# metagentools/VStrains

Measured on AMD Instinct MI355X. Metric: PE read pairs/sec through PE-link inference (GFA index + packed reads in HBM -> node_mat/short_mat), higher is better.
Workload: dtype u32

## Files before the change

vstrains_amd/csrc/vs_acc_tasks.h:

```cpp
#ifndef VS_ACC_TASKS_H
#define VS_ACC_TASKS_H
#include <stdint.h>

#include "vs_pe_plan.h"

#define VS_ACC_NODE 0u
#define VS_ACC_LEFT 1u
#define VS_ACC_RIGHT 2u

VS_PLAN_FN uint32_t vs_acc_pair_tasks(uint32_t nl, uint32_t nr) { return (nr ? nl : 0u) + ((nl + 1u) >> 1) + ((nr + 1u) >> 1); }

struct VsAccSegs {
    uint32_t p1, p2, e;
};
VS_PLAN_FN VsAccSegs vs_acc_fold(uint32_t n, uint32_t a) {
    const uint32_t a2 = n - 1u - a;
    if (a2 == a) return VsAccSegs{a, n, n};
    const bool a_first = ((0u - (n - a)) & 3u) <= ((0u - (a + 1u)) & 3u);
    return VsAccSegs{a_first ? a : a2, a_first ? a2 : a, n};
}
VS_PLAN_FN VsAccSegs vs_acc_task_segs(uint32_t kind, uint32_t a, uint32_t nl, uint32_t nr) {
    return kind == VS_ACC_NODE ? VsAccSegs{0u, nr, nr} : vs_acc_fold(kind == VS_ACC_LEFT ? nl : nr, a);
}
VS_PLAN_FN uint32_t vs_acc_turns(const VsAccSegs &s) {
    return s.p2 < s.e ? ((s.e - s.p1 + 3u) & ~3u) + (s.e - s.p2) : s.e - s.p1;
}
VS_PLAN_FN uint32_t vs_acc_partners(const VsAccSegs &s) { return (s.e - s.p1) + (s.e - s.p2); }

struct VsAccClass {
    uint32_t a0, cnt, turns;
};
VS_PLAN_FN VsAccClass vs_acc_fold_class(uint32_t n, uint32_t r) {
    const uint32_t a0 = (n - r) & 3u;
    const uint32_t pad_a = (0u - r) & 3u, pad_m = (r - n - 1u) & 3u;
    return VsAccClass{a0, ((n >> 1) + 3u - a0) >> 2, n + 1u + (pad_a <= pad_m ? pad_a : pad_m)};
}

VS_PLAN_FN uint16_t vs_acc_task_entry(uint32_t pair, uint32_t kind, uint32_t a) { return (uint16_t)(0x8000u | pair | kind << 6 | a << 8); }
VS_PLAN_FN uint32_t vs_acc_entry_pair(uint32_t w) { return w & 63u; }
VS_PLAN_FN uint32_t vs_acc_entry_kind(uint32_t w) { return (w >> 6) & 3u; }
VS_PLAN_FN uint32_t vs_acc_entry_a(uint32_t w) { return (w >> 8) & 31u; }

VS_PLAN_FN bool vs_acc_batch_fits(uint32_t tasks_incl, uint32_t cap) { return tasks_incl <= cap; }
inline uint32_t vs_acc_batch_cut(const uint32_t *tasks, uint32_t n, uint32_t first, uint32_t cap) {
    uint32_t incl = 0, last = first;
    while (last < n && vs_acc_batch_fits(incl + tasks[last], cap)) incl += tasks[last++];
    return last;
}

#endif
```

vstrains_amd/csrc/vs_api.hip:

```cpp
#include <stdarg.h>
#include <stdio.h>
#include <stdlib.h>
#include <string.h>

#include "vs_internal.h"

static thread_local std::string g_create_err;

int vs_fail(vs_ctx *ctx, int code, const char *fmt, ...) {
    char buf[512];
    va_list ap;
    va_start(ap, fmt);
    vsnprintf(buf, sizeof buf, fmt, ap);
    va_end(ap);
    if (ctx) ctx->err = buf; else g_create_err = buf;
    return code;
}

static bool env_on(const char *name) {
    const char *v = getenv(name);
    return v && atoi(v) != 0;
}

void vs_tuning_load(VsTuning &t, bool experiment) {
    t = VsTuning();
    if (!experiment) return;
    if (const char *v = getenv("VS_EPT")) t.ept = (uint32_t)atoi(v) & ~1u;
    if (const char *v = getenv("VS_GRID_PER_CU")) t.grid_per_cu = atoi(v) > 0 ? (uint32_t)atoi(v) : 128u;
    if (const char *v = getenv("VS_ACC_FILL")) t.acc_fill_pct = atoi(v);
    if (const char *v = getenv("VS_ACC_TASKS")) t.acc_tasks = atoi(v) > 0 ? (uint32_t)atoi(v) : 0u;
    if (const char *v = getenv("VS_SHORTCUT")) t.shortcut = atoi(v) != 0 ? 1 : 0;
    if (const char *v = getenv("VS_ADAPT_GRID")) t.adapt_grid = atoi(v) != 0 ? 1 : 0;
    if (const char *v = getenv("VS_ACC_ROWS")) t.acc_rows = atoi(v) != 0 ? 1 : 0;
    if (const char *v = getenv("VS_LTAB_BITS")) t.ltab_bits = atoi(v) >= 0 && atoi(v) <= 31 ? atoi(v) : -1;
    if (const char *v = getenv("VS_ROWS_KEYS")) t.rows_keys = atoi(v) >= 2 && atoi(v) <= 65536 ? (uint32_t)atoi(v) : 0u;
    if (const char *v = getenv("VS_ROWS_SUB")) t.rows_sub = atoi(v) >= 1024 ? (uint32_t)atoi(v) : 0u;
    if (const char *v = getenv("VS_ROWS_PER_STRIP")) t.rows_per_strip = atoi(v) > 0 && atoi(v) <= 64 ? (uint32_t)atoi(v) : 0u;
    t.no_sort = env_on("VS_NO_SORT");
    t.locus_global = env_on("VS_LOCUS_GLOBAL");
    t.no_fast = env_on("VS_NO_FAST");
    t.no_std = env_on("VS_NO_STD");
    t.no_agg = env_on("VS_NO_AGG");
    t.no_mid = env_on("VS_NO_MID");
}

extern "C" {

int vs_abi_version(void) { return VS_ABI_VERSION; }

int vs_device_count(void) {
    int n = 0;
    if (hipGetDeviceCount(&n) != hipSuccess) return 0;
    return n;
}

const char *vs_last_error(const vs_ctx *ctx) { return ctx ? ctx->err.c_str() : g_create_err.c_str(); }

int vs_ctx_create(int device, vs_ctx **out) {
    if (!out) return vs_fail(nullptr, VS_E_ARG, "vs_ctx_create: out is NULL");
    *out = nullptr;
    int n = 0;
    hipError_t e = hipGetDeviceCount(&n);
    if (e != hipSuccess || n <= 0)
        return vs_fail(nullptr, VS_E_HIP, "no HIP device available (%s); this library has no CPU path",
                       e == hipSuccess ? "device count 0" : hipGetErrorString(e));
    if (device < 0 || device >= n) return vs_fail(nullptr, VS_E_ARG, "device %d out of range (0..%d)", device, n - 1);
    e = hipSetDevice(device);
    if (e != hipSuccess) return vs_fail(nullptr, VS_E_HIP, "hipSetDevice(%d): %s", device, hipGetErrorString(e));
    vs_ctx *ctx = new vs_ctx();
    ctx->device = device;
    if (const char *ev = getenv("VS_EXPERIMENT")) ctx->experiment = strcmp(ev, "1") == 0;
    vs_tuning_load(ctx->tune, ctx->experiment);
    hipDeviceProp_t prop;
    if (hipGetDeviceProperties(&prop, device) == hipSuccess) ctx->n_cu = prop.multiProcessorCount;
    for (int i = 0; i < 5; i++) {
        e = hipEventCreate(&ctx->ev[i]);
        if (e != hipSuccess) {
            int rc = vs_fail(nullptr, VS_E_HIP, "hipEventCreate: %s", hipGetErrorString(e));
            delete ctx;
            return rc;
        }
    }
    *out = ctx;
// ... 162 lines not shown
```

vstrains_amd/csrc/vs_pe.hip:

```cpp
#include <stdio.h>
#include <stdlib.h>
#include <string.h>

#include <vector>

#include "vs_internal.h"
#include "vs_acc_tasks.h"
#include "vs_pe_pack.h"

#define TPB 256
#define LCAP 20u
__device__ __forceinline__ const uint32_t *vs_row_quad(const uint32_t *__restrict__ lists, const uint32_t *__restrict__ hi, uint64_t row, uint32_t q) {
    return q < LC / 4u ? lists + row * LC + 4u * q : hi + row * 4u;
}
#define EMPTY_NODE 0xFFFFFFFFu

struct PeParams {
    VsIndexDev idx;
    VsReadsDev rd;
    uint32_t *node_mat, *short_mat;
    unsigned long long *stats;
    uint32_t ept, pmax, words_cap, pool, pool_bits;
    uint64_t n_tiles;
    uint32_t *slow_list, *slow_count;
    uint32_t *dbg_lists, *dbg_counts;
    uint32_t dbg_cap;
    uint32_t accumulate;
    const uint32_t *perm;
    uint32_t wpe;
    uint32_t tiles_per_wg;
    uint32_t magic_pmax, magic_wpe;
    uint32_t *out_lists;
    uint32_t *out_counts;
    uint32_t out_rows;
    uint32_t *out_lists_hi;
    uint64_t n_pairs;
    uint32_t shortcut;
    uint8_t *tile_map;
    uint32_t tile_T;
    uint32_t mid_fast;
};

__device__ __forceinline__ void vs_mark_tile(uint8_t *map, uint32_t T, uint32_t mat, uint32_t x, uint32_t y) {
    if (!map) return;
    const uint64_t t = ((uint64_t)mat * T + (x >> 6)) * T + (y >> 6);
    if (!map[t]) map[t] = 1;
}

__device__ __forceinline__ void vs_mark_tile_store(uint8_t *map, uint32_t T, uint32_t mat, uint32_t x, uint32_t y) {
    if (map) map[((uint64_t)mat * T + (x >> 6)) * T + (y >> 6)] = 1;
}

struct Mem {
    uint32_t cnt, minp, minj;
};

struct __attribute__((packed, aligned(4))) VsQuad { uint32_t x, y, z, w; };

template <bool W4>
__device__ __forceinline__ void vs_agree_fast(const uint32_t *rw, uint32_t rbase, const uint32_t *tw, uint32_t tl, uint32_t cl,
// ... 756 lines not shown
                    P.out_counts[(uint64_t)tile * ept + i] = (s_state[i] & 3u) == 1u ? s_ns[i] : 0u;
            }
        }
        if (want_dbg) {
            for (uint32_t i = tid; i < ne; i += TTPB) {
                if (s_state[i] & 2u) continue;
                uint32_t n = s_ns[i];
                const uint64_t ge = s_gend[i];
                P.dbg_counts[ge] = n;
                for (uint32_t k2 = 0; k2 < n && k2 < P.dbg_cap; k2++) P.dbg_lists[ge * P.dbg_cap + k2] = s_list[s_off[i] + k2];
            }
        }
    }
    __syncthreads();
    if (tid < 3 && P.stats && s_misc[12 + tid]) atomicAdd(&P.stats[tid], (unsigned long long)s_misc[12 + tid]);
}

#define ACC_LDS_BYTES ((2u * ACC_SLOTS + (ACC_TPB / 64) * (ACC_TASK_WORDS + ACC_BINS) + 4u) * 4u)
static_assert(ACC_LDS_BYTES <= 160u * 1024u, "k_pe_accumulate: one workgroup per CU");
template <uint32_t BITS>
struct CellTable {
    static constexpr uint32_t EMPTY = 0xFFFFFFFFu;
    __device__ static uint32_t key(uint32_t mat, uint32_t x, uint32_t y, uint32_t N) { return (mat * N + x) * N + y; }
    __device__ static uint32_t slot(uint32_t k) { return ((((k >> 4) * 0x9E3779B1u) >> (36u - BITS)) << 4) | (k & 15u); }
    __device__ static uint32_t next(uint32_t at) { return (at + 16u) & ((1u << BITS) - 1u); }
};
typedef CellTable<ACC_BITS> Acc32;

template <typename TB>
__device__ __forceinline__ bool vs_cell_claim(uint32_t *s_key, uint32_t *s_cnt, uint32_t *s_used, uint32_t key, uint32_t at, uint32_t wgt) {
    for (uint32_t pr = 0; pr < 8u; pr++) {
        uint32_t kx = s_key[at];
        if (kx == TB::EMPTY) {
            kx = atomicCAS(&s_key[at], TB::EMPTY, key);
            if (kx == TB::EMPTY) { atomicAdd(s_used, 1u); kx = key; }
        }
        if (kx == key) {
            atomicAdd(&s_cnt[at], wgt);
            return true;
        }
        at = TB::next(at);
    }
    return false;
}

__device__ __forceinline__ void vs_wave_lds_sync() {
    __builtin_amdgcn_fence(__ATOMIC_RELEASE, "workgroup");
    __builtin_amdgcn_wave_barrier();
    __builtin_amdgcn_fence(__ATOMIC_ACQUIRE, "workgroup");
}

__global__ void __launch_bounds__(ACC_TPB)
k_pe_accumulate(const uint32_t *__restrict__ lists, const uint32_t *__restrict__ counts, uint64_t n_slots_pairs,
                uint32_t pairs_per_wg, uint32_t N, uint32_t use_table, uint32_t fill_limit, uint32_t task_cap,
                uint32_t *__restrict__ node_mat, uint32_t *__restrict__ short_mat, uint32_t *__restrict__ queue, uint32_t ept) {
    const uint32_t tid = threadIdx.x, lane = tid & 63u, wv = tid >> 6;
    uint32_t *s_key = vs_lds;
    uint32_t *s_cnt = vs_lds + ACC_SLOTS;
    uint32_t *s_bin = vs_lds + 2u * ACC_SLOTS + wv * (ACC_TASK_WORDS + ACC_BINS);
    uint16_t *s_task = (uint16_t *)(s_bin + ACC_BINS);
    uint32_t *s_misc = vs_lds + 2u * ACC_SLOTS + (ACC_TPB / 64) * (ACC_TASK_WORDS + ACC_BINS);
    uint32_t &s_used = s_misc[0], &s_lost = s_misc[1], &s_chunk = s_misc[2];
    const uint32_t NN = N * N;
    for (uint32_t i = tid; i < ACC_SLOTS; i += ACC_TPB) { s_key[i] = Acc32::EMPTY; s_cnt[i] = 0; }
    if (tid == 0) { s_used = 0; s_lost = 0; }
    __syncthreads();
    const uint32_t ppt = ept >> 1, region_q = (ept * LC) >> 2;
    auto write_out = [&]() {
        for (uint32_t i = tid; i < ACC_SLOTS; i += ACC_TPB) {
            const uint32_t key = s_key[i];
            if (key != Acc32::EMPTY) {
                atomicAdd(key >= NN ? short_mat + (key - NN) : node_mat + key, s_cnt[i]);
                s_key[i] = Acc32::EMPTY;
                s_cnt[i] = 0;
            }
        }
        if (tid == 0) { s_used = 0; s_lost = 0; }
        __syncthreads();
    };
    for (;;) {
    __syncthreads();
    if (tid == 0) s_chunk = atomicAdd(queue, 1u);
    __syncthreads();
    const uint64_t chunk = s_chunk;
    const uint64_t lo = chunk * pairs_per_wg;
    if (lo >= n_slots_pairs) break;
    const uint64_t hi = lo + pairs_per_wg < n_slots_pairs ? lo + pairs_per_wg : n_slots_pairs;
    for (uint64_t base = lo; base < hi; base += (ACC_TPB / 64u) * ACC_PPW) {
        const uint64_t wbase = base + wv * ACC_PPW;
        const uint32_t *wcounts = counts + 2u * wbase;
        const uint64_t tile0 = wbase / ppt;
        const uint32_t rem0 = (uint32_t)(wbase - tile0 * ppt);
        const uint32_t *wlists = lists + tile0 * ept * LC;
        uint32_t nl = 0, nr = 0, packed = 0;
        if (wbase + lane < hi) {
            const uint2 c = *(const uint2 *)(wcounts + 2u * lane);
            nl = c.x & 0xFFu; nr = c.y & 0xFFu;
            const uint32_t tq = (rem0 + lane) / ppt * region_q;
            packed = nl | nr << 5 | (tq + (c.x >> 8)) << 10 | (tq + (c.y >> 8)) << 21;
        }
        const uint32_t my_tasks = vs_acc_pair_tasks(nl, nr);
        for (uint32_t first = 0; first < ACC_PPW;) {
            const uint32_t incl = vs_wave_scan_add(lane >= first ? my_tasks : 0u);
            const uint32_t last = (uint32_t)__popcll(__ballot(vs_acc_batch_fits(incl, task_cap)));
            const uint32_t U = (uint32_t)__builtin_amdgcn_readlane((int)incl, (int)last - 1);
            const bool mine = lane >= first && lane < last;
            first = last;
            if (!U) continue;
            if (lane < ACC_BINS) s_bin[lane] = 0u;
            vs_wave_lds_sync();
            uint32_t o_n = 0, o_lm = 0, o_rm = 0, o_l[4], o_r[4];
            if (mine) {
                if (nl && nr) o_n = atomicAdd(&s_bin[nr], nl);
                if (nl & 1u) o_lm = atomicAdd(&s_bin[(nl + 1u) >> 1], 1u);
                if (nr & 1u) o_rm = atomicAdd(&s_bin[(nr + 1u) >> 1], 1u);
#pragma unroll
                for (uint32_t r = 0; r < 4u; r++) {
                    const VsAccClass cl = vs_acc_fold_class(nl, r), cr = vs_acc_fold_class(nr, r);
                    o_l[r] = cl.cnt ? atomicAdd(&s_bin[cl.turns], cl.cnt) : 0u;
                    o_r[r] = cr.cnt ? atomicAdd(&s_bin[cr.turns], cr.cnt) : 0u;
                }
            }
            vs_wave_lds_sync();
            {
                const uint32_t v = lane < ACC_BINS ? s_bin[ACC_BINS - 1u - lane] : 0u;
                const uint32_t before = vs_wave_scan_add(v) - v;
                if (lane < ACC_BINS) s_bin[ACC_BINS - 1u - lane] = before;
            }
            vs_wave_lds_sync();
            if (mine) {
                if (nl && nr) {
                    const uint32_t at = s_bin[nr] + o_n;
                    for (uint32_t a = 0; a < nl; a++) s_task[at + a] = vs_acc_task_entry(lane, VS_ACC_NODE, a);
                }
                if (nl & 1u) s_task[s_bin[(nl + 1u) >> 1] + o_lm] = vs_acc_task_entry(lane, VS_ACC_LEFT, nl >> 1);
                if (nr & 1u) s_task[s_bin[(nr + 1u) >> 1] + o_rm] = vs_acc_task_entry(lane, VS_ACC_RIGHT, nr >> 1);
                uint32_t nl2 = nl, nr2 = nr;
                asm volatile("" : "+v"(nl2), "+v"(nr2));
#pragma unroll
                for (uint32_t r = 0; r < 4u; r++) {
                    const VsAccClass cl = vs_acc_fold_class(nl2, r), cr = vs_acc_fold_class(nr2, r);
                    if (cl.cnt) {
                        const uint32_t at = s_bin[cl.turns] + o_l[r];
                        for (uint32_t i = 0; i < cl.cnt; i++) s_task[at + i] = vs_acc_task_entry(lane, VS_ACC_LEFT, cl.a0 + 4u * i);
                    }
                    if (cr.cnt) {
                        const uint32_t at = s_bin[cr.turns] + o_r[r];
                        for (uint32_t i = 0; i < cr.cnt; i++) s_task[at + i] = vs_acc_task_entry(lane, VS_ACC_RIGHT, cr.a0 + 4u * i);
                    }
                }
            }
            vs_wave_lds_sync();
            struct Task {
                uint32_t x, mat, off, p, p2, e, turns;
                VsQuad q;
            };
            auto decode = [&](uint32_t t0) {
                Task T;
                const uint32_t w = t0 + lane < U ? s_task[t0 + lane] : 0u;
                const uint32_t kind = vs_acc_entry_kind(w), a = vs_acc_entry_a(w);
                const uint32_t pk = __shfl(packed, (int)vs_acc_entry_pair(w), 64);
                const uint32_t ql = pk & 31u, qr = (pk >> 5) & 31u, rowl = ((pk >> 10) & 0x7FFu) << 2, rowr = (pk >> 21) << 2;
                const VsAccSegs s = w ? vs_acc_task_segs(kind, a, ql, qr) : VsAccSegs{0u, 0u, 0u};
                T.turns = vs_acc_turns(s);
                T.mat = kind != VS_ACC_NODE ? 1u : 0u;
                T.off = !w ? 0u : kind == VS_ACC_LEFT ? rowl : rowr;
                T.p = s.p1; T.p2 = s.p2; T.e = s.e;
                T.x = 0u;
                if (w && kind == VS_ACC_NODE) T.x = wlists[rowl + a];
                T.q = *(const VsQuad *)(wlists + T.off + T.p);
                return T;
            };
            Task nxt = decode(0u);
            for (uint32_t t0 = 0; t0 < U; t0 += 64u) {
                const Task c = nxt;
                if (t0 + 64u < U) nxt = decode(t0 + 64u);
                const uint32_t tmax = (uint32_t)__builtin_amdgcn_readlane((int)vs_wave_scan_max(c.turns), 63);
                const uint32_t mat = c.mat, e = c.e;
                const uint32_t *plist = wlists + c.off;
                uint32_t x = c.x, p = c.p, p2 = c.p2;
                bool fresh = true;
                VsQuad q = c.q;
                for (uint32_t t = 0; t < tmax; t += 4u) {
                    const uint32_t ys[4] = {q.x, q.y, q.z, q.w};
                    if (mat && fresh) x = ys[0];
                    const uint32_t pb = p;
                    p += 4u;
                    fresh = p >= e;
                    if (fresh) { p = p2; p2 = e; }
                    if (t + 4u < tmax) q = *(const VsQuad *)(plist + p);
                    const uint32_t left = tmax - t;
                    if (use_table) {
                        uint32_t key[4], seen[4], at[4];
#pragma unroll
                        for (uint32_t j = 0; j < 4u; j++) {
                            if (j >= left) break;
                            const uint32_t yv = ys[j];
                            const uint32_t cx = (mat && yv < x) ? yv : x, cy = (mat && yv < x) ? x : yv;
                            key[j] = Acc32::key(mat, cx, cy, N);
                            at[j] = Acc32::slot(key[j]);
                            seen[j] = s_key[at[j]];
                        }
#pragma unroll
                        for (uint32_t j = 0; j < 4u; j++) {
                            if (j >= left) break;
                            if (pb + j >= e) continue;
                            if (seen[j] == key[j]) {
                                atomicAdd(&s_cnt[at[j]], 1u);
                            } else if (!vs_cell_claim<Acc32>(s_key, s_cnt, &s_used, key[j], at[j], 1u)) {
                                atomicAdd(&s_lost, 1u);
                                atomicAdd(key[j] >= NN ? short_mat + (key[j] - NN) : node_mat + key[j], 1u);
                            }
                        }
                    } else {
#pragma unroll
                        for (uint32_t j = 0; j < 4u; j++) {
                            if (pb + j >= e) continue;
                            const uint32_t yv = ys[j];
                            const uint32_t cx = (mat && yv < x) ? yv : x, cy = (mat && yv < x) ? x : yv;
                            atomicAdd((mat ? short_mat : node_mat) + (uint64_t)cx * N + cy, 1u);
                        }
                    }
                }
            }
        }
        __syncthreads();
        const bool spill = s_used > fill_limit || s_lost > 4096u;
        __syncthreads();
        if (spill) write_out();
    }
    }
    __syncthreads();
    write_out();
}

__global__ void __launch_bounds__(256) k_mark_tiles(const uint32_t *__restrict__ lists, const uint32_t *__restrict__ counts,
                                                   uint64_t n_slots_pairs, uint8_t *__restrict__ map, uint32_t T, uint32_t ept) {
    const uint64_t p = (uint64_t)blockIdx.x * blockDim.x + threadIdx.x;
    if (p >= n_slots_pairs) return;
    const uint32_t cl = counts[2u * p], cr = counts[2u * p + 1u], nl = cl & 0xFFu, nr = cr & 0xFFu;
    if (!nl && !nr) return;
    const uint32_t *region = lists + 2u * p / ept * ept * LC, *rl = region + 4u * (cl >> 8), *rr = region + 4u * (cr >> 8);
    uint8_t *smap = map + (uint64_t)T * T;
    uint32_t tl[8], tr[8], kl = 0, kr = 0;
    bool over = false;
    auto put = [&](uint32_t (&tt)[8], uint32_t &k, uint32_t t) {
        bool seen = false;
#pragma unroll
        for (uint32_t j = 0; j < 8u; j++) seen |= j < k && tt[j] == t;
        if (seen) return;
        if (k >= 8u) { over = true; return; }
#pragma unroll
        for (uint32_t j = 0; j < 8u; j++)
            if (j == k) tt[j] = t;
        k++;
    };
#pragma unroll
    for (uint32_t j = 0; j < 8u; j++) { tl[j] = 0u; tr[j] = 0u; }
#pragma unroll
    for (uint32_t q = 0; q < LCAP / 4u; q++) {
        if (4u * q < nl) {
            const VsQuad v = *(const VsQuad *)(rl + 4u * q);
            const uint32_t e[4] = {v.x, v.y, v.z, v.w};
#pragma unroll
            for (uint32_t i = 0; i < 4u; i++)
                if (4u * q + i < nl) put(tl, kl, e[i] >> 6);
        }
        if (4u * q < nr) {
            const VsQuad v = *(const VsQuad *)(rr + 4u * q);
            const uint32_t e[4] = {v.x, v.y, v.z, v.w};
#pragma unroll
            for (uint32_t i = 0; i < 4u; i++)
                if (4u * q + i < nr) put(tr, kr, e[i] >> 6);
// ... 853 lines not shown
            for (uint32_t key_lo = 0; key_lo < N; key_lo += n_keys) {
                const uint32_t nk = N - key_lo < n_keys ? N - key_lo : n_keys;
                if (mode) hipLaunchKernelGGL(k_rows_count<1>, dim3(n_chunks1), dim3(ROWS_TPB), rl, st, sl, sh, sc, (const uint32_t *)owners, 0ull, (const uint32_t *)n_owners, key_lo, nk, row_count);
                else hipLaunchKernelGGL(k_rows_count<0>, dim3(n_chunks), dim3(ROWS_TPB), rl, st, sl, sh, sc, (const uint32_t *)nullptr, np, (const uint32_t *)nullptr, key_lo, nk, row_count);
            }
            int rc = vs_scan_u32(ctx, row_count, row_ptr, (uint64_t)N + 1u, scan_tmp, nullptr);
            if (rc) return rc;
            for (uint32_t key_lo = 0; key_lo < N; key_lo += n_keys) {
                const uint32_t nk = N - key_lo < n_keys ? N - key_lo : n_keys;
                if (mode) hipLaunchKernelGGL(k_rows_fill<1>, dim3(n_chunks1), dim3(ROWS_TPB), rl, st, sl, sh, sc, (const uint32_t *)owners, 0ull, (const uint32_t *)n_owners, (const uint32_t *)gown, key_lo, nk, (const uint32_t *)row_ptr, row_cursor, entries);
                else hipLaunchKernelGGL(k_rows_fill<0>, dim3(n_chunks), dim3(ROWS_TPB), rl, st, sl, sh, sc, (const uint32_t *)nullptr, np, (const uint32_t *)nullptr, (const uint32_t *)gown, key_lo, nk, (const uint32_t *)row_ptr, row_cursor, entries);
            }
        }
        for (int mode = 0; mode < 2; mode++) {
            const uint32_t *row_ptr = rows + 3u * mode * cap + 2u * cap;
            const uint32_t *entries = ctx->d_row_entries.as<const uint32_t>() + (mode ? np * LCAP : 0u);
            const uint32_t n_strips = (N + R - 1u) / R;
            uint32_t grid = (uint32_t)ctx->n_cu * 2u;
            if (grid > n_strips) grid = n_strips;
            uint32_t *m = mode ? d_short_mat : d_node_mat;
            const uint32_t off = (uint32_t)(((uintptr_t)m >> 2) & 15u);
            VS_HIP(ctx, hipMemsetAsync(queue, 0, sizeof(uint32_t), st));
            if (mode)
                hipLaunchKernelGGL(k_rows_sum<1>, dim3(grid), dim3(RS_TPB), RSUM_LDS_BYTES, st, sl, sh, sc, (const uint32_t *)mult, N, row_ptr, entries, R, n_strips, fill, m,
                                   off, d_tile_map, T, queue);
            else
                hipLaunchKernelGGL(k_rows_sum<0>, dim3(grid), dim3(RS_TPB), RSUM_LDS_BYTES, st, sl, sh, sc, (const uint32_t *)mult, N, row_ptr, entries, R, n_strips, fill, m,
                                   off, d_tile_map, T, queue);
        }
    }
    VS_HIP(ctx, hipGetLastError());
    return VS_OK;
}

static int pe_count_from_lists(vs_ctx *ctx, const PePlan &pl, uint32_t N, uint64_t used_ends, uint32_t *d_node_mat, uint32_t *d_short_mat,
                               uint8_t *d_tile_map) {
    hipStream_t st = ctx->stream;
    const uint32_t T = (N + 63u) >> 6;
    if (pl.list_ends > used_ends)
        VS_HIP(ctx, hipMemsetAsync(ctx->d_list_counts.as<uint32_t>() + used_ends, 0, sizeof(uint32_t) * (pl.list_ends - used_ends), st));
    const uint64_t slots_pairs = pl.list_ends / 2;
    VS_HIP(ctx, hipEventRecord(ctx->ev[4], st));
    if (pl.use_rows) {
        const int rc = pe_count_by_rows(ctx, pl, N, d_node_mat, d_short_mat, d_tile_map, T);
        if (rc) return rc;
        ctx->last_launched |= VS_RAN_ROW_OWNERS;
    } else {
        uint32_t *acc_queue = ctx->d_slow_count.as<uint32_t>() + vs_ctx::SC_ACC_QUEUE;
        if (pl.mark_tiles)
            hipLaunchKernelGGL(k_mark_tiles, dim3((unsigned)((slots_pairs + 255u) / 256u)), dim3(256), 0, st, ctx->d_lists.as<const uint32_t>(),
                               ctx->d_list_counts.as<const uint32_t>(), slots_pairs, d_tile_map, T, pl.ept);
        VS_HIP(ctx, hipFuncSetAttribute((const void *)k_pe_accumulate, hipFuncAttributeMaxDynamicSharedMemorySize, (int)ACC_LDS_BYTES));
        hipLaunchKernelGGL(k_pe_accumulate, dim3(pl.acc_grid), dim3(ACC_TPB), ACC_LDS_BYTES, st, ctx->d_lists.as<const uint32_t>(),
                           ctx->d_list_counts.as<const uint32_t>(), slots_pairs, pl.acc_per_wg, N, pl.use_table, pl.acc_fill, pl.acc_task_cap, d_node_mat,
                           d_short_mat, acc_queue, pl.ept);
    }
    return VS_OK;
}

struct TilesFn {
    uint32_t mode, sw, sp, ad;
    const void *fn;
    const char *name;
};
#define TILES(M, SW, SP) {M, SW, SP, 0u, (const void *)k_pe_tiles<M, SW, SP>, "k_pe_tiles<" #M ", " #SW ", " #SP ">"}
#define TILES_AD(M, SW, SP) {M, SW, SP, 1u, (const void *)k_pe_tiles<M, SW, SP, true>, "k_pe_tiles<" #M ", " #SW ", " #SP ", true>"}, TILES(M, SW, SP)
static const TilesFn TILES_TABLE[] = {TILES_AD(1, 10u, 4u), TILES_AD(1, 8u, 3u), TILES_AD(1, 7u, 2u), TILES_AD(1, 7u, 3u), TILES(1, 0u, 0u),
                                      TILES_AD(2, 16u, 2u), TILES(2, 0u, 0u),    TILES(0, 0u, 0u)};

static int pe_launch(vs_ctx *ctx, const vs_reads *reads, uint32_t *d_node_mat, uint32_t *d_short_mat, uint64_t *d_stats,
                     uint32_t *d_dbg_lists, uint32_t *d_dbg_counts, uint32_t dbg_cap, uint8_t *d_tile_map = nullptr) {
    if (!ctx->has_index) return vs_fail(ctx, VS_E_STATE, "vs_pe_count: build an index first (vs_index_build)");
    VS_HIP(ctx, hipSetDevice(ctx->device));
    hipStream_t st = ctx->stream;
    const VsIndexDev &idx = ctx->idx;
    const uint64_t n_pairs = reads->n_ends / 2;
    ctx->last_ms[0] = ctx->last_ms[1] = ctx->last_ms[2] = 0;
    ctx->last_launched = 0;
    ctx->last_order_pairs = 0;
    if (ctx->experiment) vs_tuning_load(ctx->tune, true);
    PePlanIn in;
    in.n_nodes = idx.n_nodes; in.K = idx.K; in.w = idx.w; in.s = idx.s;
    in.n_seed_pos = ctx->n_seed_pos; in.n_distinct = ctx->n_distinct; in.max_node_len = ctx->max_node_len; in.n_cu = (uint32_t)ctx->n_cu;
    in.n_ends = reads->n_ends; in.max_len = (uint32_t)reads->max_len;
    in.has_mask = reads->d_mask != nullptr; in.has_inv4 = reads->d_inv4 != nullptr;
    in.count = d_node_mat != nullptr; in.tile_map = d_tile_map != nullptr;
    in.tune = ctx->tune;
    const PePlan pl = vs_pe_plan(in);
    if (pl.status != VS_OK) return vs_fail(ctx, pl.status, "%s", pl.msg);
    if (!pl.n_tiles) return VS_OK;
    const TilesFn *tf = nullptr;
    for (const TilesFn &t : TILES_TABLE)
        if (t.mode == pl.mode && t.sw == pl.sw && t.sp == pl.sp && t.ad == pl.ad) tf = &t;
    if (!tf) return vs_fail(ctx, VS_E_STATE, "vs_pe_count: the plan names k_pe_tiles<%u, %uu, %uu, %u>, which this build does not hold", pl.mode, pl.sw, pl.sp, pl.ad);

    VS_HIP(ctx, ctx->d_slow_list.reserve(sizeof(uint32_t) * n_pairs));
    VS_HIP(ctx, ctx->d_slow_count.reserve(sizeof(uint32_t) * vs_ctx::SC_WORDS));
    VS_HIP(ctx, ctx->d_slow_list2.reserve(sizeof(uint32_t) * n_pairs));
    if (ctx->dense_nodes != idx.n_nodes) ctx->d_dense.reset();
    bool dense_new = false;
    VS_HIP(ctx, ctx->d_dense.reserve(pl.dense_bytes, pl.dense_bytes, &dense_new));
    if (dense_new) {
        ctx->dense_nodes = idx.n_nodes;
        uint64_t N = idx.n_nodes ? idx.n_nodes : 1;
        VS_HIP(ctx, hipMemsetAsync(ctx->d_dense.ptr(), 0xFF, pl.dense_bytes, st));
        hipLaunchKernelGGL(k_dense_zero_cnt, dim3((unsigned)((N * pl.slow_grid + TPB - 1) / TPB)), dim3(TPB), 0, st,
                           ctx->d_dense.as<uint32_t>(), N, (uint64_t)pl.slow_grid);
// ... 245 lines not shown
```

vstrains_amd/csrc/vs_pe_plan.h:

```cpp
#ifndef VS_PE_PLAN_H
#define VS_PE_PLAN_H
#include <stddef.h>
#include <stdint.h>
#include <stdio.h>

#include <initializer_list>

#include "../../include/vstrains_hip.h"

#if defined(__HIPCC__)
#define VS_PLAN_FN __host__ __device__ inline
#else
#define VS_PLAN_FN inline
#endif

struct VsTuning {
    uint32_t ept = 0;
    uint32_t grid_per_cu = 128;
    int acc_fill_pct = -1;
    uint32_t acc_tasks = 0;
    int shortcut = -1;
    int adapt_grid = -1;
    int acc_rows = -1;
    int ltab_bits = -1;
    uint32_t rows_keys = 0, rows_sub = 0;
    uint32_t rows_per_strip = 0;
    bool no_sort = false, locus_global = false, no_fast = false, no_std = false, no_agg = false;
    bool no_mid = false;
};

VS_PLAN_FN uint32_t vs_seed_phase(uint32_t len, uint32_t w, uint32_t s) {
    return len < w ? 0u : ((len - w) % s + s) / 2u;
}
VS_PLAN_FN uint32_t vs_seed_probes(uint32_t len, uint32_t w, uint32_t s) {
    if (len < w) return 0u;
    return (len - w + 1u) / s;
}
#define VS_SEED_VERIFIED(w) ((w) <= 31u ? (w) : 0u)

#define LC 16u
#define PPT 2u
#define TTPB 256
#define PPT_LONG 1u
#define CHUNK (TTPB * PPT)
#define ACC_TPB 1024
#define ACC_BITS 14
#define ACC_SLOTS (1u << ACC_BITS)
#define ACC_PPW 64u
#define ACC_TASK_WORDS 480u
#define ACC_TASK_CAP (2u * ACC_TASK_WORDS)
#define ACC_TASK_MIN 40u
#define ACC_BINS 24u
#define ROWS_KEYS 65536u
#define ROWS_SUB ((1u << 26) - 1024u)
#define RS_BITS 13
#define RS_SLOTS (1u << RS_BITS)
#define LOCUS_LDS_KEYS 36864u
#define LOCUS_LDS_MAX_PASSES 4u
#define LOCUS_WGS 256u
#define SLOW_WORDS_PER_NODE 6u
#define LDS_BUDGET_BYTES (64u * 1024u)
#define NI_CAP 4096u

struct TileLayout {
    uint32_t woff, gend, meta, inv, words, pcnt, pa, pb, hkey, hcnt, hminp, hminj, ns, state, list, owner, misc, total;
};
VS_PLAN_FN TileLayout tile_layout(uint32_t ept, uint32_t pmax, uint32_t words_cap, uint32_t pool, uint32_t list_trim = 0u) {
    TileLayout t;
    uint32_t o = 0;
    const uint32_t NI = ept * pmax;
    t.woff = o;  o += 2u * ((ept + 2u) & ~1u);
    t.gend = o;  o += 2u * ept;
    t.meta = o;  o += 2u * ept;
    t.inv = o;   o += ept;
    t.words = o; o += 2u * (words_cap + 8u);
    t.pcnt = o;  o += NI + 1u;
    t.pa = o;    o += NI;
    t.pb = o;    o += NI;
    t.hkey = o;  o += pool;
    t.hcnt = o;  o += pool;
    t.hminp = o; o += pool;
    t.hminj = o; o += pool;
    t.ns = o;    o += ept;
    t.state = o; o += ept;
    t.list = o;
    t.owner = o; o += (ept * LC - list_trim > CHUNK ? ept * LC - list_trim : CHUNK);
    t.misc = o;  o += 16u;
    t.total = o;
    return t;
}

#define STD_EPT (TTPB / 4u)
#define STD_POOL_BITS 10u
#define STD_K 56u
#define STD_W 31u
#define STD_S 26u
#define STD2_EPT 60u
#define STD2_POOL_BITS 10u
#define STD2_K 128u
#define STD2_W 63u
#define STD2_S 66u
struct StdShape {
    uint32_t mode, sw, sp;
};
constexpr StdShape VS_STD_SHAPES[] = {{1u, 10u, 4u}, {1u, 8u, 3u}, {1u, 7u, 2u}, {1u, 7u, 3u}, {2u, 16u, 2u}};
struct StdTable {
    uint32_t pool, trim;
};
VS_PLAN_FN constexpr StdTable vs_std_table(int mode, bool std_shape, bool ad) {
    return std_shape && !ad ? StdTable{768u, mode == 2 ? 192u : 64u} : StdTable{1u << (mode == 2 ? STD2_POOL_BITS : STD_POOL_BITS), 0u};
}

inline uint32_t slow_grid_for(uint32_t n_nodes) {
    const uint64_t per_wg = sizeof(uint32_t) * (uint64_t)SLOW_WORDS_PER_NODE * (n_nodes ? n_nodes : 1u);
    uint64_t g = (4ull << 30) / per_wg;
    return (uint32_t)(g < 64u ? 64u : g > 2048u ? 2048u : g);
}

inline uint32_t pool_for(uint32_t ept, uint32_t *bits) {
    uint32_t b = 6;
    while ((1u << b) < 16u * ept) b++;
    *bits = b;
    return 1u << b;
}

inline size_t lds_bytes(uint32_t ept, uint32_t pmax, uint32_t words_cap) {
    uint32_t bits;
    uint32_t pool = pool_for(ept, &bits);
    return (size_t)tile_layout(ept, pmax, words_cap, pool).total * sizeof(uint32_t);
}

struct PePlanIn {
    uint32_t n_nodes = 0, K = 0, w = 0, s = 0;
    uint64_t n_seed_pos = 0, n_distinct = 0;
    uint32_t max_node_len = 0, n_cu = 0;
    uint64_t n_ends = 0;
    uint32_t max_len = 0;
    bool has_mask = false, has_inv4 = false;
    bool count = false, tile_map = false;
    VsTuning tune;
};

struct PePlan {
    int status;
    char msg[128];
    uint32_t ept, pmax, wpe, pool, pool_bits, words_cap, magic_pmax, magic_wpe;
    uint64_t lds_bytes;
    uint32_t mode, sw, sp, ad;
    uint64_t n_tiles, grid, list_ends, list_words;
    uint32_t tiles_per_wg, shortcut, mid_fast;
    uint32_t use_sort, lds_sort, locus_chunk, locus_per_pass;
    uint64_t locus_keys, locus_hist_words;
    uint32_t use_rows, use_table, mark_tiles;
    uint32_t acc_grid, acc_per_wg, acc_fill, acc_task_cap;
    uint64_t rows_sub_pairs;
    uint32_t rows_ltab_bits, rows_keys, rows_fill, rows_per_strip;
    uint32_t slow_grid;
    uint64_t dense_bytes;
};

inline PePlan vs_pe_plan(const PePlanIn &in) {
    PePlan p = {};
    const VsTuning &tn = in.tune;
    const uint64_t n_pairs = in.n_ends / 2;
    if (n_pairs == 0) return p;
    const uint32_t maxlen = in.max_len, N = in.n_nodes;
    if (N > 0x01FFFFFEu) {
        p.status = VS_E_RANGE;
        snprintf(p.msg, sizeof p.msg, "more than 2^25-2 nodes");
        return p;
    }
    const uint32_t wpe = maxlen ? (maxlen + 15u) / 16u : 1u;
    uint32_t pmax = vs_seed_probes(maxlen, in.w, in.s);
    if (!pmax) pmax = 1u;
    uint32_t ept = tn.ept ? tn.ept : STD_EPT;
    if (ept < 2 || ept > TTPB / 2u) ept = STD_EPT;
    while (ept > 2 && (ept * pmax > NI_CAP || lds_bytes(ept, pmax, ept * wpe) > LDS_BUDGET_BYTES)) ept -= 2;
    if (!tn.ept) {
        for (size_t fit : {(size_t)32000, (size_t)40000}) {
            uint32_t e2 = ept;
            while (e2 > STD_EPT / 2u && lds_bytes(e2, pmax, e2 * wpe) > fit) e2 -= 2;
            if (lds_bytes(e2, pmax, e2 * wpe) <= fit) { ept = e2; break; }
        }
    }
    size_t lds = lds_bytes(ept, pmax, ept * wpe);
    if (lds > 160u * 1024u) {
        p.status = VS_E_RANGE;
        snprintf(p.msg, sizeof p.msg, "reads of %u bases with k+1=%u need %zu B of LDS per pair (limit 160 KiB)", maxlen, in.K, lds);
        return p;
    }
    p.ept = ept;
    p.pmax = pmax;
    p.wpe = wpe;
    p.words_cap = ept * wpe;
    p.pool = pool_for(ept, &p.pool_bits);
    p.magic_pmax = pmax > 1u ? (uint32_t)(0x100000000ull / pmax) + 1u : 0u;
    p.magic_wpe = wpe > 1u ? (uint32_t)(0x100000000ull / wpe) + 1u : 0u;
    p.slow_grid = slow_grid_for(N);
    p.dense_bytes = sizeof(uint32_t) * (uint64_t)SLOW_WORDS_PER_NODE * (N ? N : 1) * p.slow_grid;

    p.use_sort = !tn.no_sort && n_pairs >= 4096 && n_pairs < 0xFFFFFFF0ull;
    if (p.use_sort) {
        const uint64_t nk = (uint64_t)N + 2u;
        const bool fits_lds = nk <= LOCUS_LDS_MAX_PASSES * LOCUS_LDS_KEYS;
        p.locus_keys = nk;
        p.locus_hist_words = fits_lds ? nk * LOCUS_WGS : nk;
        p.lds_sort = fits_lds && !tn.locus_global;
// ... 5 lines not shown

    p.use_table = tn.no_agg ? 0u : 1u;
    const bool fits32 = 2ull * N * N < 0xFFFFFFFFull;
    bool use_rows = tn.acc_rows >= 0 ? tn.acc_rows != 0 : !fits32;
    if (N == 0 || !p.use_table) use_rows = false;
    if (!use_rows && !fits32) p.use_table = 0u;
    p.use_rows = use_rows;
    p.n_tiles = (n_pairs + ept / 2 - 1) / (ept / 2);
    p.list_ends = p.n_tiles * ept;
    p.list_words = p.list_ends * (use_rows ? LC + 4u : LC) + 16u;

    p.shortcut = in.n_distinct && in.n_seed_pos < 2 * in.n_distinct ? 1u : 0u;
    if (tn.shortcut >= 0) p.shortcut = (uint32_t)tn.shortcut;
    if (VS_SEED_VERIFIED(in.w) == 0u) p.shortcut = 0u;

    const bool straight = (!in.has_mask || in.has_inv4) && in.max_node_len < (1u << 23) && !tn.no_fast;
    const bool fast = straight && in.s <= 32u && maxlen <= 128u + in.w + 32u;
    p.mid_fast = fast && VS_SEED_VERIFIED(in.w) ? 1u : 0u;
    uint32_t long_reach = 0;
    for (uint32_t len = in.K; len <= maxlen; len++) {
        const uint32_t behind = len - vs_seed_phase(len, in.w, in.s) - VS_SEED_VERIFIED(in.w);
        long_reach = behind > long_reach ? behind : long_reach;
    }
    const bool fast_long = !fast && straight && in.s <= 128u && long_reach <= 256u && maxlen < 512u;
    p.mode = fast ? 1u : fast_long ? 2u : 0u;
    const bool shape1 = p.mode == 1u && ept == STD_EPT && p.pool_bits == STD_POOL_BITS && maxlen <= 159u && in.K == STD_K && in.w == STD_W && in.s == STD_S;
    const bool shape2 = p.mode == 2u && ept == STD2_EPT && p.pool_bits == STD2_POOL_BITS && in.K == STD2_K && in.w == STD2_W && in.s == STD2_S;
    if (in.count && !tn.no_std && (shape1 || shape2))
        for (const StdShape &sh : VS_STD_SHAPES)
            if (sh.mode == p.mode && sh.sw == wpe && sh.sp == pmax) { p.sw = wpe; p.sp = pmax; }
    if (p.sw) {
        p.ad = tn.adapt_grid >= 0 ? tn.adapt_grid != 0 : in.n_distinct && in.n_seed_pos >= 6u * in.n_distinct;
        const StdTable tab = vs_std_table((int)p.mode, true, p.ad);
        lds = (size_t)tile_layout(ept, pmax, ept * wpe, tab.pool, tab.trim).total * sizeof(uint32_t);
    }
    p.lds_bytes = lds;
    const uint64_t max_grid = (uint64_t)in.n_cu * tn.grid_per_cu;
    p.grid = p.n_tiles < max_grid ? p.n_tiles : max_grid;
    p.tiles_per_wg = (uint32_t)((p.n_tiles + p.grid - 1) / p.grid);
    p.grid = (p.n_tiles + p.tiles_per_wg - 1) / p.tiles_per_wg;
    if (!in.count) return p;

    const uint64_t slots_pairs = p.list_ends / 2;
    if (!use_rows) {
        p.mark_tiles = in.tile_map;
        p.acc_grid = in.n_cu * 32u;
        p.acc_per_wg = (uint32_t)((slots_pairs + p.acc_grid - 1) / p.acc_grid);
        p.acc_per_wg = (p.acc_per_wg + ACC_TPB - 1) / ACC_TPB * ACC_TPB;
        p.acc_grid = (uint32_t)((slots_pairs + p.acc_per_wg - 1) / p.acc_per_wg);
        if (p.acc_grid > in.n_cu * 2u) p.acc_grid = in.n_cu * 2u;
        p.acc_fill = ACC_SLOTS / 16u;
        if (tn.acc_fill_pct >= 0) p.acc_fill = (uint32_t)((uint64_t)ACC_SLOTS * (uint32_t)tn.acc_fill_pct / 100u);
        p.acc_task_cap = tn.acc_tasks >= ACC_TASK_MIN && tn.acc_tasks < ACC_TASK_CAP ? tn.acc_tasks : ACC_TASK_CAP;
        return p;
    }
    const uint64_t sub_max = tn.rows_sub ? (uint64_t)tn.rows_sub : (uint64_t)ROWS_SUB;
    p.rows_sub_pairs = slots_pairs < sub_max ? slots_pairs : sub_max;
    p.rows_ltab_bits = 10;
    while ((1ull << p.rows_ltab_bits) < 2u * p.rows_sub_pairs && p.rows_ltab_bits < 31u) p.rows_ltab_bits++;
    if (tn.ltab_bits >= 0) p.rows_ltab_bits = (uint32_t)tn.ltab_bits;
    const uint32_t keys_max = tn.rows_keys ? tn.rows_keys : ROWS_KEYS;
    p.rows_keys = N < keys_max ? N : keys_max;
    p.rows_fill = RS_SLOTS / 2u;
    if (tn.acc_fill_pct >= 0) p.rows_fill = (uint32_t)((uint64_t)RS_SLOTS * (uint32_t)tn.acc_fill_pct / 100u);
    if (p.rows_fill > RS_SLOTS - 1024u) p.rows_fill = RS_SLOTS - 1024u;
    p.rows_per_strip = tn.rows_per_strip ? tn.rows_per_strip : 2u;
    return p;
}

#endif
```

Before: 1.412 billion.

## Deduplicate identical short node lists per workgroup and accumulate weighted counts

Adds an LDS hash table in the accumulate kernel that fingerprints each read end's node list (up to 8 nodes) and merges identical sets within a workgroup. Only one owner per duplicate group emits the left/right self-pair tasks, with an atomic weight equal to the multiplicity, so fewer pair-expansion tasks are scheduled. The cost is extra per-workgroup hashing, set comparison, barriers and LDS table clearing, plus possible contention on the hash table. Merging is enabled by default through the plan unless disabled by env.

```diff
diff --git a/vstrains_amd/csrc/vs_acc_merge.h b/vstrains_amd/csrc/vs_acc_merge.h
--- /dev/null
+++ b/vstrains_amd/csrc/vs_acc_merge.h
@@ -0,0 +1,138 @@
+#ifndef VS_ACC_MERGE_H
+#define VS_ACC_MERGE_H
+#include <stdint.h>
+
+#include "vs_pe_plan.h"
+
+#define VS_MERGE_PROBES 8u
+#define VS_MERGE_ONE 0x80000u
+#define VS_MERGE_NO_SLOT 0xFFFFFFFFu
+#ifndef VS_MERGE_MAX_LEN
+#define VS_MERGE_MAX_LEN 8u
+#endif
+VS_PLAN_FN bool vs_merge_enters(uint32_t n, uint32_t max_len) { return n != 0u && n <= max_len; }
+
+struct VsMergeQuad {
+    uint32_t v[4];
+};
+VS_PLAN_FN uint32_t vs_merge_quad_len(uint32_t n, uint32_t q) { return n <= q ? 0u : n - q < 4u ? n - q : 4u; }
+
+VS_PLAN_FN uint32_t vs_merge_node_hash(uint32_t v) {
+    uint32_t h = v * 0x9E3779B1u;
+    h ^= h >> 15;
+    return h * 0x2C1B3C6Du;
+}
+VS_PLAN_FN uint32_t vs_merge_quad_sum(const VsMergeQuad &a, uint32_t m) {
+    uint32_t f = 0u;
+    for (uint32_t j = 0; j < 4u; j++) f += j < m ? vs_merge_node_hash(a.v[j]) : 0u;
+    return f;
+}
+template <typename LD>
+VS_PLAN_FN uint32_t vs_merge_fingerprint(const LD &load, const uint32_t *list, uint32_t n) {
+    uint32_t f = n * 0x85EBCA6Bu;
+    const VsMergeQuad a0 = load(list, vs_merge_quad_len(n, 0u));
+    if (n > 4u) {
+        const VsMergeQuad a1 = load(list + 4, vs_merge_quad_len(n, 4u));
+        f += vs_merge_quad_sum(a1, vs_merge_quad_len(n, 4u));
+        for (uint32_t q = 8u; q < n; q += 4u) f += vs_merge_quad_sum(load(list + q, vs_merge_quad_len(n, q)), vs_merge_quad_len(n, q));
+    }
+    return f + vs_merge_quad_sum(a0, vs_merge_quad_len(n, 0u));
+}
+VS_PLAN_FN uint32_t vs_merge_slot(uint32_t f, uint32_t bits) { return ((f ^ f >> 16) * 0x9E3779B1u) >> (32u - bits); }
+VS_PLAN_FN uint32_t vs_merge_next(uint32_t at, uint32_t bits) { return (at + 1u) & ((1u << bits) - 1u); }
+
+VS_PLAN_FN uint32_t vs_merge_word(uint32_t n, uint32_t where, uint32_t weight) { return n | where << 5 | weight << 19; }
+VS_PLAN_FN uint32_t vs_merge_word_n(uint32_t w) { return w & 31u; }
+VS_PLAN_FN uint32_t vs_merge_word_where(uint32_t w) { return (w >> 5) & 0x3FFFu; }
+VS_PLAN_FN uint32_t vs_merge_word_weight(uint32_t w) { return w >> 19; }
+
+VS_PLAN_FN uint32_t vs_merge_quad_hits(const VsMergeQuad &a, uint32_t ma, const VsMergeQuad &b, uint32_t mb) {
+    const uint32_t a0 = a.v[0], a1 = ma > 1u ? a.v[1] : a0, a2 = ma > 2u ? a.v[2] : a0, a3 = ma > 3u ? a.v[3] : a0;
+    uint32_t hits = 0u;
+    for (uint32_t j = 0; j < 4u; j++) {
+        const uint32_t y = b.v[j];
+        hits += (j < mb && (y == a0 || y == a1 || y == a2 || y == a3)) ? 1u : 0u;
+    }
+    return hits;
+}
+template <typename LD>
+VS_PLAN_FN bool vs_merge_same_set(const LD &load, const uint32_t *a, const uint32_t *b, uint32_t n) {
+    uint32_t hits = 0u;
+    if (n <= 8u) {
+        const uint32_t m0 = vs_merge_quad_len(n, 0u), m1 = vs_merge_quad_len(n, 4u);
+        const VsMergeQuad a0 = load(a, m0), b0 = load(b, m0);
+        hits = vs_merge_quad_hits(a0, m0, b0, m0);
+        if (m1) {
+            const VsMergeQuad a1 = load(a + 4, m1), b1 = load(b + 4, m1);
+            hits += vs_merge_quad_hits(a0, m0, b1, m1) + vs_merge_quad_hits(a1, m1, b0, m0) + vs_merge_quad_hits(a1, m1, b1, m1);
+        }
+        return hits == n;
+    }
+    for (uint32_t qa = 0; qa < n; qa += 4u) {
+        const uint32_t ma = vs_merge_quad_len(n, qa);
+        const VsMergeQuad aq = load(a + qa, ma);
+        for (uint32_t qb = 0; qb < n; qb += 4u) hits += vs_merge_quad_hits(aq, ma, load(b + qb, vs_merge_quad_len(n, qb)), vs_merge_quad_len(n, qb));
+    }
+    return hits == n;
+}
+
+template <typename T, typename LD, typename L>
+VS_PLAN_FN uint32_t vs_merge_enter(T &tab, const LD &load, const L &list_at, uint32_t bits, uint32_t where, const uint32_t *mine, uint32_t n, uint32_t f, uint32_t *ordinal) {
+    uint32_t at = vs_merge_slot(f, bits);
+    *ordinal = 0u;
+    for (uint32_t pr = 0; pr < VS_MERGE_PROBES; pr++) {
+        uint32_t w = tab.load(at);
+        if (w == 0u) {
+            w = tab.cas(at, vs_merge_word(n, where, 1u));
+            if (w == 0u) return at;
+        }
+        if (vs_merge_word_n(w) == n && vs_merge_same_set(load, mine, list_at(vs_merge_word_where(w)), n)) {
+            *ordinal = vs_merge_word_weight(tab.add(at, VS_MERGE_ONE));
+            return at;
+        }
+        at = vs_merge_next(at, bits);
+    }
+    return VS_MERGE_NO_SLOT;
+}
+VS_PLAN_FN uint32_t vs_merge_weight(uint32_t word, uint32_t ordinal, uint32_t f) {
+    const uint32_t weight = vs_merge_word_weight(word);
+    const uint32_t owner = (uint32_t)(((uint64_t)(f * 0x9E3779B1u) * weight) >> 32);
+    return ordinal == owner ? weight : 0u;
+}
+
+struct VsMergeHostTable {
+    uint32_t *w;
+    uint32_t load(uint32_t at) { return w[at]; }
+    uint32_t cas(uint32_t at, uint32_t word) {
+        const uint32_t old = w[at];
+        if (old == 0u) w[at] = word;
+        return old;
+    }
+    uint32_t add(uint32_t at, uint32_t v) {
+        const uint32_t old = w[at];
+        w[at] = old + v;
+        return old;
+    }
+};
+struct VsMergeHostLoad {
+    VsMergeQuad operator()(const uint32_t *p, uint32_t m) const {
+        VsMergeQuad a = {{0u, 0u, 0u, 0u}};
+        for (uint32_t j = 0; j < m; j++) a.v[j] = p[j];
+        return a;
+    }
+};
+inline void vs_merge_round(const uint32_t *const *lists, const uint32_t *n, uint32_t n_ends, uint32_t bits, uint32_t max_len, uint32_t *table, uint32_t *weight) {
+    for (uint32_t i = 0; i < (1u << bits); i++) table[i] = 0u;
+    VsMergeHostTable tab{table};
+    auto list_at = [&](uint32_t end) { return lists[end]; };
+    const VsMergeHostLoad load;
+    uint32_t slot[2048], ordinal[2048];
+    for (uint32_t e = 0; e < n_ends; e++) {
+        slot[e] = VS_MERGE_NO_SLOT;
+        if (vs_merge_enters(n[e], max_len)) slot[e] = vs_merge_enter(tab, load, list_at, bits, e, lists[e], n[e], vs_merge_fingerprint(load, lists[e], n[e]), &ordinal[e]);
+    }
+    for (uint32_t e = 0; e < n_ends; e++)
+        weight[e] = !n[e] ? 0u : slot[e] == VS_MERGE_NO_SLOT ? 1u : vs_merge_weight(table[slot[e]], ordinal[e], vs_merge_fingerprint(load, lists[e], n[e]));
+}
+
+#endif
diff --git a/vstrains_amd/csrc/vs_acc_tasks.h b/vstrains_amd/csrc/vs_acc_tasks.h
--- a/vstrains_amd/csrc/vs_acc_tasks.h
+++ b/vstrains_amd/csrc/vs_acc_tasks.h
@@ -9,6 +9,9 @@
 #define VS_ACC_RIGHT 2u
 
 VS_PLAN_FN uint32_t vs_acc_pair_tasks(uint32_t nl, uint32_t nr) { return (nr ? nl : 0u) + ((nl + 1u) >> 1) + ((nr + 1u) >> 1); }
+VS_PLAN_FN uint32_t vs_acc_merged_tasks(uint32_t nl, uint32_t nr, bool node, bool left, bool right) {
+    return (node && nr ? nl : 0u) + (left ? (nl + 1u) >> 1 : 0u) + (right ? (nr + 1u) >> 1 : 0u);
+}
 
 struct VsAccSegs {
     uint32_t p1, p2, e;
diff --git a/vstrains_amd/csrc/vs_api.hip b/vstrains_amd/csrc/vs_api.hip
--- a/vstrains_amd/csrc/vs_api.hip
+++ b/vstrains_amd/csrc/vs_api.hip
@@ -29,6 +29,8 @@
     if (const char *v = getenv("VS_GRID_PER_CU")) t.grid_per_cu = atoi(v) > 0 ? (uint32_t)atoi(v) : 128u;
     if (const char *v = getenv("VS_ACC_FILL")) t.acc_fill_pct = atoi(v);
     if (const char *v = getenv("VS_ACC_TASKS")) t.acc_tasks = atoi(v) > 0 ? (uint32_t)atoi(v) : 0u;
+    if (const char *v = getenv("VS_ACC_MERGE")) t.acc_merge = atoi(v) != 0 ? 1 : 0;
+    if (const char *v = getenv("VS_ACC_LBITS")) t.acc_lbits = atoi(v) > 0 ? (uint32_t)atoi(v) : 0u;
     if (const char *v = getenv("VS_SHORTCUT")) t.shortcut = atoi(v) != 0 ? 1 : 0;
     if (const char *v = getenv("VS_ADAPT_GRID")) t.adapt_grid = atoi(v) != 0 ? 1 : 0;
     if (const char *v = getenv("VS_ACC_ROWS")) t.acc_rows = atoi(v) != 0 ? 1 : 0;
diff --git a/vstrains_amd/csrc/vs_pe.hip b/vstrains_amd/csrc/vs_pe.hip
--- a/vstrains_amd/csrc/vs_pe.hip
+++ b/vstrains_amd/csrc/vs_pe.hip
@@ -6,6 +6,7 @@
 
 #include "vs_internal.h"
 #include "vs_acc_tasks.h"
+#include "vs_acc_merge.h"
 #include "vs_pe_pack.h"
 
 #define TPB 256
@@ -868,7 +869,7 @@
 
 __global__ void __launch_bounds__(ACC_TPB)
 k_pe_accumulate(const uint32_t *__restrict__ lists, const uint32_t *__restrict__ counts, uint64_t n_slots_pairs,
-                uint32_t pairs_per_wg, uint32_t N, uint32_t use_table, uint32_t fill_limit, uint32_t task_cap,
+                uint32_t pairs_per_wg, uint32_t N, uint32_t use_table, uint32_t fill_limit, uint32_t task_cap, uint32_t merge_bits,
                 uint32_t *__restrict__ node_mat, uint32_t *__restrict__ short_mat, uint32_t *__restrict__ queue, uint32_t ept) {
     const uint32_t tid = threadIdx.x, lane = tid & 63u, wv = tid >> 6;
     uint32_t *s_key = vs_lds;
@@ -915,8 +916,45 @@
             const uint32_t tq = (rem0 + lane) / ppt * region_q;
             packed = nl | nr << 5 | (tq + (c.x >> 8)) << 10 | (tq + (c.y >> 8)) << 21;
         }
-        const uint32_t my_tasks = vs_acc_pair_tasks(nl, nr);
+        uint32_t wts = (nl ? 1u << 22 : 0u) | (nr ? 1u << 23 : 0u);
+        if (merge_bits) {
+            uint32_t *s_tab = vs_lds + 2u * ACC_SLOTS;
+            for (uint32_t i = tid; i < (1u << merge_bits); i += ACC_TPB) s_tab[i] = 0u;
+            const uint64_t rtile0 = base / ppt;
+            const uint32_t *rlists = lists + rtile0 * ept * LC;
+            const uint32_t wq = (uint32_t)(tile0 - rtile0) * region_q;
+            const uint32_t ql = wq + ((packed >> 10) & 0x7FFu), qr = wq + (packed >> 21);
+            auto load = [](const uint32_t *p, uint32_t) {
+                const VsQuad q = *(const VsQuad *)p;
+                return VsMergeQuad{{q.x, q.y, q.z, q.w}};
+            };
+            const bool ml = vs_merge_enters(nl, VS_MERGE_MAX_LEN), mr = vs_merge_enters(nr, VS_MERGE_MAX_LEN);
+            const uint32_t fl = ml ? vs_merge_fingerprint(load, rlists + (ql << 2), nl) : 0u, fr = mr ? vs_merge_fingerprint(load, rlists + (qr << 2), nr) : 0u;
+            __syncthreads();
+            struct {
+                uint32_t *w;
+                __device__ uint32_t load(uint32_t at) { return __atomic_load_n(&w[at], __ATOMIC_RELAXED); }
+                __device__ uint32_t cas(uint32_t at, uint32_t word) { return atomicCAS(&w[at], 0u, word); }
+                __device__ uint32_t add(uint32_t at, uint32_t v) { return atomicAdd(&w[at], v); }
+            } tab{s_tab};
+            auto list_at = [&](uint32_t quad) { return rlists + (quad << 2); };
+            uint32_t slot_l = VS_MERGE_NO_SLOT, slot_r = VS_MERGE_NO_SLOT, ord_l = 0u, ord_r = 0u;
+            if (ml) slot_l = vs_merge_enter(tab, load, list_at, merge_bits, ql, rlists + (ql << 2), nl, fl, &ord_l);
+            if (mr) slot_r = vs_merge_enter(tab, load, list_at, merge_bits, qr, rlists + (qr << 2), nr, fr, &ord_r);
+            __syncthreads();
+            uint32_t wl = nl ? 1u : 0u, wr = nr ? 1u : 0u;
+            if (slot_l != VS_MERGE_NO_SLOT) wl = vs_merge_weight(s_tab[slot_l], ord_l, fl);
+            if (slot_r != VS_MERGE_NO_SLOT) wr = vs_merge_weight(s_tab[slot_r], ord_r, fr);
+            wts = wl ? (wl - 1u) | 1u << 22 : 0u;
+            if (wr) wts |= (wr - 1u) << 11 | 1u << 23;
+            __syncthreads();
+        }
         for (uint32_t first = 0; first < ACC_PPW;) {
+            uint32_t pk0 = packed, ws0 = wts;
+            asm volatile("" : "+v"(pk0), "+v"(ws0));
+            const uint32_t nl = pk0 & 31u, nr = (pk0 >> 5) & 31u;
+            const uint32_t sl = ws0 & 1u << 22 ? nl : 0u, sr = ws0 & 1u << 23 ? nr : 0u;
+            const uint32_t my_tasks = vs_acc_merged_tasks(nl, nr, true, sl != 0u, sr != 0u);
             const uint32_t incl = vs_wave_scan_add(lane >= first ? my_tasks : 0u);
             const uint32_t last = (uint32_t)__popcll(__ballot(vs_acc_batch_fits(incl, task_cap)));
             const uint32_t U = (uint32_t)__builtin_amdgcn_readlane((int)incl, (int)last - 1);
@@ -928,11 +966,11 @@
             uint32_t o_n = 0, o_lm = 0, o_rm = 0, o_l[4], o_r[4];
             if (mine) {
                 if (nl && nr) o_n = atomicAdd(&s_bin[nr], nl);
-                if (nl & 1u) o_lm = atomicAdd(&s_bin[(nl + 1u) >> 1], 1u);
-                if (nr & 1u) o_rm = atomicAdd(&s_bin[(nr + 1u) >> 1], 1u);
+                if (sl & 1u) o_lm = atomicAdd(&s_bin[(sl + 1u) >> 1], 1u);
+                if (sr & 1u) o_rm = atomicAdd(&s_bin[(sr + 1u) >> 1], 1u);
 #pragma unroll
                 for (uint32_t r = 0; r < 4u; r++) {
-                    const VsAccClass cl = vs_acc_fold_class(nl, r), cr = vs_acc_fold_class(nr, r);
+                    const VsAccClass cl = vs_acc_fold_class(sl, r), cr = vs_acc_fold_class(sr, r);
                     o_l[r] = cl.cnt ? atomicAdd(&s_bin[cl.turns], cl.cnt) : 0u;
                     o_r[r] = cr.cnt ? atomicAdd(&s_bin[cr.turns], cr.cnt) : 0u;
                 }
@@ -949,9 +987,9 @@
                     const uint32_t at = s_bin[nr] + o_n;
                     for (uint32_t a = 0; a < nl; a++) s_task[at + a] = vs_acc_task_entry(lane, VS_ACC_NODE, a);
                 }
-                if (nl & 1u) s_task[s_bin[(nl + 1u) >> 1] + o_lm] = vs_acc_task_entry(lane, VS_ACC_LEFT, nl >> 1);
-                if (nr & 1u) s_task[s_bin[(nr + 1u) >> 1] + o_rm] = vs_acc_task_entry(lane, VS_ACC_RIGHT, nr >> 1);
-                uint32_t nl2 = nl, nr2 = nr;
+                if (sl & 1u) s_task[s_bin[(sl + 1u) >> 1] + o_lm] = vs_acc_task_entry(lane, VS_ACC_LEFT, sl >> 1);
+                if (sr & 1u) s_task[s_bin[(sr + 1u) >> 1] + o_rm] = vs_acc_task_entry(lane, VS_ACC_RIGHT, sr >> 1);
+                uint32_t nl2 = sl, nr2 = sr;
                 asm volatile("" : "+v"(nl2), "+v"(nr2));
 #pragma unroll
                 for (uint32_t r = 0; r < 4u; r++) {
@@ -968,7 +1006,7 @@
             }
             vs_wave_lds_sync();
             struct Task {
-                uint32_t x, mat, off, p, p2, e, turns;
+                uint32_t x, mw, off, p, p2, e, turns;
                 VsQuad q;
             };
             auto decode = [&](uint32_t t0) {
@@ -976,10 +1014,11 @@
                 const uint32_t w = t0 + lane < U ? s_task[t0 + lane] : 0u;
                 const uint32_t kind = vs_acc_entry_kind(w), a = vs_acc_entry_a(w);
                 const uint32_t pk = __shfl(packed, (int)vs_acc_entry_pair(w), 64);
+                const uint32_t ws = __shfl(wts, (int)vs_acc_entry_pair(w), 64);
                 const uint32_t ql = pk & 31u, qr = (pk >> 5) & 31u, rowl = ((pk >> 10) & 0x7FFu) << 2, rowr = (pk >> 21) << 2;
                 const VsAccSegs s = w ? vs_acc_task_segs(kind, a, ql, qr) : VsAccSegs{0u, 0u, 0u};
                 T.turns = vs_acc_turns(s);
-                T.mat = kind != VS_ACC_NODE ? 1u : 0u;
+                T.mw = kind == VS_ACC_NODE ? 2u : 3u + (((kind == VS_ACC_LEFT ? ws : ws >> 11) & 0x7FFu) << 1);
                 T.off = !w ? 0u : kind == VS_ACC_LEFT ? rowl : rowr;
                 T.p = s.p1; T.p2 = s.p2; T.e = s.e;
                 T.x = 0u;
@@ -992,7 +1031,7 @@
                 const Task c = nxt;
                 if (t0 + 64u < U) nxt = decode(t0 + 64u);
                 const uint32_t tmax = (uint32_t)__builtin_amdgcn_readlane((int)vs_wave_scan_max(c.turns), 63);
-                const uint32_t mat = c.mat, e = c.e;
+                const uint32_t mat = c.mw & 1u, wgt = c.mw >> 1, e = c.e;
                 const uint32_t *plist = wlists + c.off;
                 uint32_t x = c.x, p = c.p, p2 = c.p2;
                 bool fresh = true;
@@ -1022,10 +1061,10 @@
                             if (j >= left) break;
                             if (pb + j >= e) continue;
                             if (seen[j] == key[j]) {
-                                atomicAdd(&s_cnt[at[j]], 1u);
-                            } else if (!vs_cell_claim<Acc32>(s_key, s_cnt, &s_used, key[j], at[j], 1u)) {
+                                atomicAdd(&s_cnt[at[j]], wgt);
+                            } else if (!vs_cell_claim<Acc32>(s_key, s_cnt, &s_used, key[j], at[j], wgt)) {
                                 atomicAdd(&s_lost, 1u);
-                                atomicAdd(key[j] >= NN ? short_mat + (key[j] - NN) : node_mat + key[j], 1u);
+                                atomicAdd(key[j] >= NN ? short_mat + (key[j] - NN) : node_mat + key[j], wgt);
                             }
                         }
                     } else {
@@ -1034,7 +1073,7 @@
                             if (pb + j >= e) continue;
                             const uint32_t yv = ys[j];
                             const uint32_t cx = (mat && yv < x) ? yv : x, cy = (mat && yv < x) ? x : yv;
-                            atomicAdd((mat ? short_mat : node_mat) + (uint64_t)cx * N + cy, 1u);
+                            atomicAdd((mat ? short_mat : node_mat) + (uint64_t)cx * N + cy, wgt);
                         }
                     }
                 }
@@ -1994,7 +2033,7 @@
                                ctx->d_list_counts.as<const uint32_t>(), slots_pairs, d_tile_map, T, pl.ept);
         VS_HIP(ctx, hipFuncSetAttribute((const void *)k_pe_accumulate, hipFuncAttributeMaxDynamicSharedMemorySize, (int)ACC_LDS_BYTES));
         hipLaunchKernelGGL(k_pe_accumulate, dim3(pl.acc_grid), dim3(ACC_TPB), ACC_LDS_BYTES, st, ctx->d_lists.as<const uint32_t>(),
-                           ctx->d_list_counts.as<const uint32_t>(), slots_pairs, pl.acc_per_wg, N, pl.use_table, pl.acc_fill, pl.acc_task_cap, d_node_mat,
+                           ctx->d_list_counts.as<const uint32_t>(), slots_pairs, pl.acc_per_wg, N, pl.use_table, pl.acc_fill, pl.acc_task_cap, pl.acc_merge_bits, d_node_mat,
                            d_short_mat, acc_queue, pl.ept);
     }
     return VS_OK;
diff --git a/vstrains_amd/csrc/vs_pe_plan.h b/vstrains_amd/csrc/vs_pe_plan.h
--- a/vstrains_amd/csrc/vs_pe_plan.h
+++ b/vstrains_amd/csrc/vs_pe_plan.h
@@ -19,6 +19,8 @@
     uint32_t grid_per_cu = 128;
     int acc_fill_pct = -1;
     uint32_t acc_tasks = 0;
+    int acc_merge = -1;
+    uint32_t acc_lbits = 0;
     int shortcut = -1;
     int adapt_grid = -1;
     int acc_rows = -1;
@@ -50,6 +52,7 @@
 #define ACC_TASK_WORDS 480u
 #define ACC_TASK_CAP (2u * ACC_TASK_WORDS)
 #define ACC_TASK_MIN 40u
+#define ACC_MERGE_BITS 12u
 #define ACC_BINS 24u
 #define ROWS_KEYS 65536u
 #define ROWS_SUB ((1u << 26) - 1024u)
@@ -153,6 +156,7 @@
     uint64_t locus_keys, locus_hist_words;
     uint32_t use_rows, use_table, mark_tiles;
     uint32_t acc_grid, acc_per_wg, acc_fill, acc_task_cap;
+    uint32_t acc_merge_bits;
     uint64_t rows_sub_pairs;
     uint32_t rows_ltab_bits, rows_keys, rows_fill, rows_per_strip;
     uint32_t slow_grid;
@@ -264,6 +268,7 @@
         p.acc_fill = ACC_SLOTS / 16u;
         if (tn.acc_fill_pct >= 0) p.acc_fill = (uint32_t)((uint64_t)ACC_SLOTS * (uint32_t)tn.acc_fill_pct / 100u);
         p.acc_task_cap = tn.acc_tasks >= ACC_TASK_MIN && tn.acc_tasks < ACC_TASK_CAP ? tn.acc_tasks : ACC_TASK_CAP;
+        p.acc_merge_bits = tn.acc_merge == 0 ? 0u : tn.acc_lbits >= 1u && tn.acc_lbits < ACC_MERGE_BITS ? tn.acc_lbits : ACC_MERGE_BITS;
         return p;
     }
     const uint64_t sub_max = tn.rows_sub ? (uint64_t)tn.rows_sub : (uint64_t)ROWS_SUB;
```

Result: faster. 1.433 billion (median of 6 runs) (+1.5%).
